# ShannonAI/GNN-LM

Hardware: AMD Instinct MI355X
Metric: eval tokens/sec on WikiText-103 (k=1024, GNN+KNN); test ppl match (higher is better)
Workload: dtype f32

## Files before the change

### gnn-lm_amd/csrc/ivfpq_mfma.hip

```cpp
#include "kernels.h"

namespace gnnlm {
namespace {

typedef int v4i __attribute__((ext_vector_type(4)));
typedef int v8i __attribute__((ext_vector_type(8)));
typedef unsigned u32x2 __attribute__((ext_vector_type(2)));
typedef unsigned v4u __attribute__((ext_vector_type(4)));
constexpr int QG = 8;
constexpr int TAB_BYTES = 2 * 256 * 32 * QG;
#ifndef GNNLM_IVF8_WAVE_CAP
#define GNNLM_IVF8_WAVE_CAP 240
#endif
constexpr int WAVE_CAP = GNNLM_IVF8_WAVE_CAP;
constexpr int SCAN_CTL = 768;
constexpr int SCAN_LDS = TAB_BYTES + SCAN_CTL + 16 * WAVE_CAP * 8;
static_assert(SCAN_LDS <= 160 * 1024, "the filter's tables + staging regions exceed a CU's LDS");
constexpr int HIST_BINS = 1024, HIST_SHIFT = 4;
constexpr int SUMS_LDS = TAB_BYTES + QG * HIST_BINS * 4;
constexpr int SURV_CNT_STRIDE = 16;
constexpr int QLUT_BYTES = 64 * 256;
constexpr int SURV_ROW_BITS = 19, SURV_LIST_BITS = 18, SURV_EXCESS_MAX = 254, SURV_SUM_BIG = 16383;

__global__ __launch_bounds__(256) void pack_tiles_kernel(const uint8_t* __restrict__ codes, int64_t N, uint8_t* __restrict__ out) {
// ... 381 lines not shown
                    const uint32_t t0 = GNNLM_PERM(b, a, 0x05010400u), t1 = GNNLM_PERM(b, a, 0x07030602u);
                    const uint32_t t2 = GNNLM_PERM(d, c, 0x05010400u), t3 = GNNLM_PERM(d, c, 0x07030602u);
                    o[0 + hq] = GNNLM_PERM(t2, t0, 0x05040100u);
                    o[2 + hq] = GNNLM_PERM(t2, t0, 0x07060302u);
                    o[4 + hq] = GNNLM_PERM(t3, t1, 0x05040100u);
                    o[6 + hq] = GNNLM_PERM(t3, t1, 0x07060302u);
                }
                uint4* dst = reinterpret_cast<uint4*>(smem) + 2 * (tid + (i0 + it) * NTH);
                dst[0] = uint4{o[0], o[1], o[2], o[3]};
                dst[1] = uint4{o[4], o[5], o[6], o[7]};
            }
        }
    }
#endif
    const int j = lane & 15, g = lane >> 4;
    const int qs_lane = lane < QG ? gq[lane] : -1;
    uint32_t* hist = reinterpret_cast<uint32_t*>(smem + TAB_BYTES);
    if (SUMS) for (int e = tid; e < QG * HIST_BINS; e += NTH) hist[e] = 0u;
    constexpr int T_NEVER = 16384;
    int T4[4] = {T_NEVER, T_NEVER, T_NEVER, T_NEVER};
    uint32_t *hist_a = nullptr, *hist_b = nullptr;
    if (SUMS) {
        const int q0 = 4 * (g & 1) + (g >= 2 ? 2 : 0) + (j & 1), q1 = q0 ^ 1;
        if (gq[q0] >= 0 && p.grp_out[(int64_t)grp * QG + q0] >= 0) hist_a = hist + q0 * HIST_BINS;
        if (gq[q1] >= 0 && p.grp_out[(int64_t)grp * QG + q1] >= 0) hist_b = hist + q1 * HIST_BINS;
    } else if (g < 2) {
#pragma unroll
        for (int r = 0; r < 4; ++r) {
            const int qr = gq[4 * g + r];
            if (qr >= 0) T4[r] = max(-T_NEVER, min(T_NEVER, filter_threshold(p.qmeta, qr, p.coarse[(int64_t)qr * p.ld_coarse + list], p.tau[qr])));
        }
    }
#if GNNLM_IVF8_EXP & 32
    if (p.cap > 0) T4[0] = T4[1] = T4[2] = T4[3] = T_NEVER;
#elif GNNLM_IVF8_EXP & 255
    T4[0] = T4[1] = T4[2] = T4[3] = T_NEVER;
#endif
    if (!SUMS && wave == 0) {
        int Tl = 0;
#pragma unroll
        for (int sl = 0; sl < QG; ++sl) {
            const int t = __builtin_amdgcn_readlane(T4[sl & 3], 16 * (sl >> 2));
            if (lane == sl) Tl = t;
        }
        if (lane < QG) { wgc[lane] = 0; wgc[8 + lane] = Tl; wgc[16 + lane] = qs_lane; }
    }
    const v4i negT = SUMS ? v4i{0, 0, 0, 0} : v4i{1 - T4[0], 1 - T4[1], 1 - T4[2], 1 - T4[3]};
    __syncthreads();
    phase(0);
#if GNNLM_IVF8_EXP & 1024
    const long long g0 = clock64();
#endif

    uint32_t tc[8];
#pragma unroll
    for (int s = 0; s < 8; ++s) {
        const uint32_t s0 = (uint32_t)(16 * (g & 1) + ((j + 2 * s) & 15)) << 3, s1 = (uint32_t)(16 * (g & 1) + ((j + 2 * s + 1) & 15)) << 3;
        tc[s] = s0 | s1 << 8 | (uint32_t)(g >> 1) << 16;
    }
    uint32_t sel[4] = {0u, 0u, 0u, 0u}, sidx = 0xccccccccu;
    if (j < QG) {
        const int pos = j & 3;
#pragma unroll
        for (int h = 0; h < 2; ++h)
#pragma unroll
            for (int lk = 0; lk < 2; ++lk) {
                const int s0 = 8 * h + 2 * (2 * lk + (j >> 2));
                const int sb = pos < 3 ? s0 : s0 + 1;
                sel[sb >> 2] |= 1u << (8 * (sb & 3));
                if (pos < 3) sidx = (sidx & ~(3u << (2 * s0))) | (uint32_t)pos << (2 * s0);
            }
    }
    const v4i Asel = {(int)sel[0], (int)sel[1], (int)sel[2], (int)sel[3]};

    const int64_t t_lo = lo >> 4;
    const int nt = (int)(((hi - 1) >> 4) - t_lo) + 1;
    const int len = (int)(hi - lo), row_shift = (int)(lo & 15);
    const __amdgpu_buffer_rsrc_t rs = __builtin_amdgcn_make_buffer_rsrc(const_cast<uint8_t*>(p.tiles) + t_lo * 1024, 0, nt * 1024, 0x00020000);
    const int wv = __builtin_amdgcn_readfirstlane(wave);
    const int voff = lane * 16;
    const uint32_t rs_lane = (uint32_t)((j - row_shift) * 8) + (uint32_t)(4 * (g & 1));
    auto load_tile = [&](int u) -> v4u {
#if GNNLM_IVF8_EXP & 1
        return v4u{(uint32_t)u * 2654435761u + lane, (uint32_t)u * 40503u ^ lane, (uint32_t)u + 77u * lane, (uint32_t)u * 3u + lane};
#elif GNNLM_IVF8_EXP & 256
        return __builtin_amdgcn_raw_buffer_load_b128(rs, voff, __builtin_amdgcn_readfirstlane((u & 3) * 1024), 0);
#else
        return __builtin_amdgcn_raw_buffer_load_b128(rs, voff, __builtin_amdgcn_readfirstlane(u * 1024), 0);
#endif
    };
    auto lookups4 = [&](const v4u& cw, int q, v8i& X) __attribute__((always_inline)) {
        const uint32_t w[4] = {cw.x, cw.y, cw.z, cw.w};
#pragma unroll
        for (int e = 0; e < 4; ++e) {
            const int pp = 4 * q + e;
            const uint32_t ad = GNNLM_PERM(w[pp >> 2], tc[pp >> 1], 0x0c020000u | (uint32_t)(4 + (pp & 3)) << 8 | (uint32_t)(pp & 1));
#if GNNLM_IVF8_EXP & 4
            const u32x2 x = u32x2{ad, ad ^ 0x55u};
#else
            const u32x2 x = *reinterpret_cast<const __attribute__((address_space(3))) u32x2*>(ad);
#endif
            X[2 * e] = (int)x.x;
            X[2 * e + 1] = (int)x.y;
        }
    };
    int wcnt = 0;
    auto count_entries = [&](int* ctr) __attribute__((always_inline)) {
        for (int c = lane; c < wcnt; c += 64) {
            const uint2 e = wbuf[c];
#pragma unroll
            for (int r = 0; r < 4; ++r)
                if (e.y >> (8 * r) & 255u) atomicAdd(&ctr[(e.x & 4u) + r], 1);
        }
    };
    auto write_entries = [&](int* pos) __attribute__((always_inline)) {
        for (int c = lane; c < wcnt; c += 64) {
            const uint2 e = wbuf[c];
            const uint32_t row = (uint32_t)(lo + ((e.x >> 3) & ((1u << SURV_ROW_BITS) - 1u)));
#pragma unroll
            for (int r = 0; r < 4; ++r) {
                const int b8 = (int)(e.y >> (8 * r) & 255u);
                if (b8 == 0) continue;
                const int sl = (int)(e.x & 4u) + r;
                const int64_t at = atomicAdd(&pos[sl], 1);
                const int Tsl = wgc[8 + sl], qsl = wgc[16 + sl];
                if (at < p.cap && qsl >= 0) {
                    const int ex = b8 - 1;
                    const int su = ex >= SURV_EXCESS_MAX ? SURV_SUM_BIG : min(SURV_SUM_BIG - 1, max(0, ex + Tsl + 128 * 64));
                    surv[(int64_t)qsl * p.cap + at] = uint2{row, (uint32_t)list | (uint32_t)su << SURV_LIST_BITS};
                }
            }
        }
        wcnt = 0;
    };
    auto flush_wave = [&]() __attribute__((always_inline)) {
        if (wcnt == 0) return;
        if (lane < QG) wc[lane] = 0;
        count_entries(wc);
        if (lane < QG) {
            const int tot = wc[lane];
            wc[lane] = (tot > 0 && qs_lane >= 0) ? atomicAdd(&p.surv_cnt[(int64_t)qs_lane * SURV_CNT_STRIDE], tot) : 0;
        }
        write_entries(wc);
    };
    constexpr int PF = SUMS ? GNNLM_IVF8_PF_SUMS : GNNLM_IVF8_PF;
    v8i X[4];
    const int TS = SUMS ? max(1, p.sums_stride) : 1;
    auto step = [&](const v4u& cn, v4u& cl, int u) __attribute__((always_inline)) {
        tick(-1);
        cl = load_tile(u + PF * NW * TS);
        v4i acc = negT;
#pragma unroll
        for (int q = 0; q < 4; ++q) {
#if GNNLM_IVF8_EXP & 8
            acc += v4i{X[q][0], X[q][1], X[q][2], X[q][3]} + v4i{X[q][4], X[q][5], X[q][6], X[q][7]};
#else
            acc = __builtin_amdgcn_smfmac_i32_16x16x128_i8(Asel, X[q], acc, (int)sidx, 0, 0);
#endif
            lookups4(cn, q, X[q]);
            __builtin_amdgcn_sched_barrier(0);
        }
        tick(0);
        const int row = 16 * u + j - row_shift;
        const bool edge = u == 0 || u >= nt - 1;
        if (SUMS) {
            const gnnlm_u32x2 w2 = __builtin_amdgcn_permlane32_swap((uint32_t)acc[2], (uint32_t)acc[2], false, false);
            const gnnlm_u32x2 w3 = __builtin_amdgcn_permlane32_swap((uint32_t)acc[3], (uint32_t)acc[3], false, false);
            const int e0 = g >= 2 ? (int)w2.x : acc[0], e1 = g >= 2 ? (int)w3.x : acc[1];
            const int s0 = (j & 1) ? e1 : e0, s1 = (j & 1) ? e0 : e1;
            if (!edge || (unsigned)row < (unsigned)len) {
                if (hist_a) atomicAdd(&hist_a[(s0 + 128 * 64) >> HIST_SHIFT], 1u);
                if (hist_b) atomicAdd(&hist_b[(s1 + 128 * 64) >> HIST_SHIFT], 1u);
            }
        } else {
            if (wcnt + 32 > WAVE_CAP) flush_wave();
            tick(1);
            uint32_t lo8, hi8;
            const uint32_t p01 = GNNLM_PERM((uint32_t)acc[1], (uint32_t)acc[0], 0x05040100u), p23 = GNNLM_PERM((uint32_t)acc[3], (uint32_t)acc[2], 0x05040100u);
            asm("v_sat_pk_u8_i16 %0, %1" : "=v"(lo8) : "v"(p01));
            asm("v_sat_pk_u8_i16 %0, %1" : "=v"(hi8) : "v"(p23));
            const uint32_t ex4 = GNNLM_PERM(hi8, lo8, 0x05040100u);
            const uint32_t rowslot = ((uint32_t)(16 * u) << 3) + rs_lane;
            const uint32_t lim = edge ? (uint32_t)len << 3 : 0xffffffffu;
            uint32_t ex4r = rowslot < lim ? ex4 : 0u;
            asm("" : "+v"(ex4r));
            const bool keep = ex4r != 0u;
            const uint64_t m = __builtin_amdgcn_ballot_w64(keep);
            const int rank = __builtin_amdgcn_mbcnt_hi((uint32_t)(m >> 32), __builtin_amdgcn_mbcnt_lo((uint32_t)m, 0u));
            if (keep) wbuf[wcnt + rank] = uint2{rowslot, ex4r};
            wcnt = __builtin_amdgcn_readfirstlane(wcnt + __builtin_popcountll(m));
            tick(2);
        }
    };
    {
        int u = SUMS ? wv * TS + list % TS : wv;
        v4u C[PF];
#pragma unroll
        for (int i = 0; i < PF; ++i) C[i] = load_tile(u + i * NW * TS);
#pragma unroll
        for (int q = 0; q < 4; ++q) lookups4(C[0], q, X[q]);
#define GNNLM_IVF8_STEP(t) if constexpr (PF > (t)) { step(C[((t) + 1) % PF], C[(t)], u); u += NW * TS; }
        while (u < nt) {
            GNNLM_IVF8_STEP(0) GNNLM_IVF8_STEP(1) GNNLM_IVF8_STEP(2) GNNLM_IVF8_STEP(3)
            GNNLM_IVF8_STEP(4) GNNLM_IVF8_STEP(5) GNNLM_IVF8_STEP(6) GNNLM_IVF8_STEP(7)
        }
#undef GNNLM_IVF8_STEP
        static_assert(PF >= 3 && PF <= 8, "GNNLM_IVF8_PF");
        phase(1);
#if GNNLM_IVF8_EXP & 512
        if (tid == 512 && p.work_ctr) for (int i = 0; i < 3; ++i) { atomicAdd(&p.work_ctr[(blockIdx.x & 7) * 16 + 8 + i], acc_t[i]); acc_t[i] = 0; }
        if (tid == 512 && p.work_ctr) atomicAdd(&p.work_ctr[(blockIdx.x & 7) * 16 + 11], (nt - wv + NW - 1) / NW);
#endif
#if GNNLM_IVF8_EXP & 1024
        if (lane == 0 && p.work_ctr) atomicAdd(&p.work_ctr[(blockIdx.x & 7) * 16 + (wave ? wave : 15)], (int)((clock64() - g0) >> 4));
#endif
    }
    if (SUMS) {
        __syncthreads();
#pragma unroll
        for (int u = 0; u < QG; ++u) {
            const int64_t ob = p.grp_out[(int64_t)grp * QG + u];
            if (qs[u] < 0 || ob < 0) continue;
            for (int e = tid; e < HIST_BINS; e += NTH) p.out_hist[ob + e] = hist[u * HIST_BINS + e];
        }
        advance_slow();
        continue;
    }
    count_entries(wgc);
    if (tid == 0) *next_s = next_index();
    phase(3);
    __syncthreads();
    phase(4);
    if (tid < QG) {
        const int tot = wgc[tid];
        wgc[tid] = (tot > 0 && qs_lane >= 0) ? atomicAdd(&p.surv_cnt[(int64_t)qs_lane * SURV_CNT_STRIDE], tot) : 0;
    }
    __syncthreads();
    gi_next = *next_s;
    phase(5);
    write_entries(wgc);
    }
#if GNNLM_IVF8_EXP & 512
    if (tid == 0 && p.work_ctr) {
        atomicAdd(&p.work_ctr[(blockIdx.x & 7) * 16 + 12], (int)((clock64() - k0) >> 4));
        atomicAdd(&p.work_ctr[(blockIdx.x & 7) * 16 + 13], (int)(wall_clock64() - w0));
    }
#endif
}

__global__ __launch_bounds__(1024) void ivfpq_tau_kernel(gnnlm_ivfpq_tau_t p) {
    constexpr int CB = 2 * HIST_BINS;
    __shared__ int comb[CB];
    __shared__ int part[1024];
    __shared__ int bstar_s;
    const int tid = threadIdx.x;
    const int64_t q = blockIdx.x;
    const float delta = p.qmeta[q * 4], sum_lo = p.qmeta[q * 4 + 1], amax = p.qmeta[q * 4 + 2];
    float bmin = INFINITY, bmax = -INFINITY;
    for (int d = 0; d < p.D; ++d) {
        if (p.probe_list[q * p.ld_probe + d] < 0) continue;
        const float b = p.probe_bias[q * p.ld_probe + d];
        bmin = fminf(bmin, b);
        bmax = fmaxf(bmax, b);
    }
    int c0 = 0, c1 = 0;
    for (int d = 0; d < p.D; ++d) {
        if (p.probe_list[q * p.ld_probe + d] < 0) continue;
        const float offf = (p.probe_bias[q * p.ld_probe + d] - bmin) / delta * 0.9999f - 1.f;
        const int sh = (int)fminf(fmaxf(offf, 0.f), (float)(HIST_BINS << HIST_SHIFT)) >> HIST_SHIFT;
        const uint32_t* h = p.hist + (q * p.D + d) * HIST_BINS;
        const int b0 = tid - sh, b1 = tid + 1024 - sh;
        if (b0 >= 0 && b0 < HIST_BINS) c0 += (int)h[b0];
        if (b1 >= 0 && b1 < HIST_BINS) c1 += (int)h[b1];
    }
    comb[tid] = c0;
    comb[tid + 1024] = c1;
    if (tid == 0) bstar_s = -1;
    __syncthreads();
    const int h0 = comb[2 * tid], h1 = comb[2 * tid + 1], mine = h0 + h1;
    part[tid] = mine;
    __syncthreads();
    int suf = mine;
    for (int step = 1; step < 1024; step <<= 1) {
        const int other = tid + step < 1024 ? part[tid + step] : 0;
        __syncthreads();
        suf += other;
        part[tid] = suf;
        __syncthreads();
    }
    if (suf >= p.k && suf - mine < p.k) bstar_s = (suf - mine + h1 >= p.k) ? 2 * tid + 1 : 2 * tid;
    __syncthreads();
    if (tid == 0) {
        float tau = -INFINITY;
        if (bstar_s >= 0) {
            const float eps = 66.f * 2.3841858e-7f * (64.f * amax + fmaxf(fabsf(bmin), fabsf(bmax)));
            tau = (bmin + sum_lo) + (float)(bstar_s << HIST_SHIFT) * delta * (1.f - 6.1035156e-5f) - eps;
            tau -= fabsf(tau) * 2.3841858e-7f + 1e-30f;
        }
        p.tau[q] = tau;
    }
}

#ifndef GNNLM_REFINE_NT
#define GNNLM_REFINE_NT 1024
#endif
struct RefineParams {
    uint32_t* surv;  const int32_t* surv_cnt;  int32_t* out_cnt;  int32_t cap;
    float* tau;  const float* qmeta;
    const float* coarse;  int64_t ld_coarse;
    int64_t n;  int32_t k;
};
template <int EPT>
__device__ __forceinline__ void refine_wg(const RefineParams& p, const int64_t q, int* hist, int& n_left, float& tau_left) {
    constexpr int NT = GNNLM_REFINE_NT, NB = 2048, NWV = NT / 64;
    __shared__ int wtot[NWV];
    __shared__ int dig_s, base_s;
    const int tid = threadIdx.x, lane = tid & 63, wave = tid >> 6;
    const int n = min(p.surv_cnt[q * SURV_CNT_STRIDE], p.cap);
    uint2* surv = reinterpret_cast<uint2*>(p.surv) + q * p.cap;
    const float tau0 = p.tau[q];
    n_left = n;
    tau_left = tau0;
    if (n < p.k || !(tau0 > -INFINITY)) {
        if (tid == 0 && p.out_cnt) p.out_cnt[q * SURV_CNT_STRIDE] = n;
        return;
    }
    const float delta = p.qmeta[q * 4], sum_lo = p.qmeta[q * 4 + 1], amax = p.qmeta[q * 4 + 2];
    const float dlo = delta * (1.f - 6.1035156e-5f);
    const float* coarse = p.coarse + q * p.ld_coarse;
    auto lower_bound = [&](const uint2& rec) -> float {
        const int list = (int)(rec.y & ((1u << SURV_LIST_BITS) - 1u));
        int su = (int)(rec.y >> SURV_LIST_BITS);
        const float bias = coarse[list];
        if (su >= SURV_SUM_BIG) su = min(16320, max(0, filter_threshold(p.qmeta, q, bias, tau0) + SURV_EXCESS_MAX + 128 * 64));
        const float eps = 66.f * 2.3841858e-7f * (64.f * amax + fabsf(bias));
        const float lb = (bias + sum_lo) + (float)su * dlo - eps;
        return lb - (fabsf(lb) * 2.3841858e-7f + 1e-30f);
    };
    constexpr int C0 = EPT * NT;
    uint2 rrec[EPT];
    float rlb[EPT];
#pragma unroll
    for (int e = 0; e < EPT; ++e) rrec[e] = surv[min(tid + e * NT, n - 1)];
    float mx = -INFINITY;
#pragma unroll
    for (int e = 0; e < EPT; ++e) {
        rlb[e] = tid + e * NT < n ? lower_bound(rrec[e]) : -INFINITY;
        mx = fmaxf(mx, rlb[e]);
    }
    for (int c = C0 + tid; c < n; c += NT) mx = fmaxf(mx, lower_bound(surv[c]));
    __shared__ float wmax[NWV];
    mx = wave_max(mx);
    if (lane == 0) wmax[wave] = mx;
    __syncthreads();
    mx = wmax[0];
    for (int w = 1; w < NWV; ++w) mx = fmaxf(mx, wmax[w]);
    const float span = mx - tau0;
    float tau1 = tau0;
    if (span > 0.f) {
        const float inv_w = (float)NB / span * (1.f - 1e-6f);
        for (int e = tid; e < NB; e += NT) hist[e] = 0;
        __syncthreads();
        auto bin_of = [&](float lb) -> int { return lb >= tau0 ? min(NB - 1, (int)((lb - tau0) * inv_w)) : -1; };
#pragma unroll
        for (int e = 0; e < EPT; ++e) {
            const int bn = bin_of(rlb[e]);
            if (bn >= 0) atomicAdd(&hist[bn], 1);
        }
        for (int c = C0 + tid; c < n; c += NT) {
            const int bn = bin_of(lower_bound(surv[c]));
            if (bn >= 0) atomicAdd(&hist[bn], 1);
        }
        __syncthreads();
        constexpr int BPT = NB / NT;
        int own[BPT], mine = 0;
#pragma unroll
        for (int bb = 0; bb < BPT; ++bb) { own[bb] = hist[BPT * tid + bb]; mine += own[bb]; }
        int suf = mine;
#pragma unroll
        for (int d = 1; d < 64; d <<= 1) {
            const int o = __shfl_down(suf, d, 64);
            if (lane + d < 64) suf += o;
        }
        if (lane == 0) wtot[wave] = suf;
        if (tid == 0) dig_s = -1;
        __syncthreads();
        for (int w = wave + 1; w < NWV; ++w) suf += wtot[w];
        if (suf >= p.k && suf - mine < p.k) {
            int acc_ = suf - mine;
#pragma unroll
            for (int bb = BPT - 1; bb >= 0; --bb) {
                if (acc_ + own[bb] >= p.k) { dig_s = BPT * tid + bb; break; }
                acc_ += own[bb];
            }
        }
        __syncthreads();
        if (dig_s > 0) {
            const float t = tau0 + (float)dig_s / inv_w * (1.f - 2e-6f);
            tau1 = fmaxf(tau0, t - fabsf(t) * 4.7683716e-7f);
        }
    }
    auto keep_rec = [&](const uint2& rec) -> bool {
        const int list = (int)(rec.y & ((1u << SURV_LIST_BITS) - 1u)), su = (int)(rec.y >> SURV_LIST_BITS);
        if (su >= SURV_SUM_BIG) return true;
        const float bias = coarse[list];
        const float eps = 66.f * 2.3841858e-7f * (64.f * amax + fabsf(bias) + fabsf(tau1));
        const float ub = (bias + sum_lo) + (float)(su + 66) * delta * 1.001f + eps;
        return !(ub < tau1);
    };
    int kept = 0;
    uint32_t kmask = 0u;
#pragma unroll
    for (int e = 0; e < EPT; ++e)
        if (tid + e * NT < n && keep_rec(rrec[e])) { kmask |= 1u << e; ++kept; }
    int incl = kept;
#pragma unroll
    for (int d = 1; d < 64; d <<= 1) {
        const int o = __shfl_up(incl, d, 64);
        if (lane >= d) incl += o;
    }
    __syncthreads();
    if (lane == 63) wtot[wave] = incl;
    __syncthreads();
    int at = incl - kept;
    for (int w = 0; w < wave; ++w) at += wtot[w];
    int total = 0;
    for (int w = 0; w < NWV; ++w) total += wtot[w];
#pragma unroll
    for (int e = 0; e < EPT; ++e)
        if (kmask >> e & 1u) surv[at++] = rrec[e];
    if (n > C0) {
        if (tid == 0) base_s = total;
        __syncthreads();
        for (int c0 = C0; c0 < n; c0 += NT) {
            const int c = c0 + tid;
            uint2 rec = uint2{0u, 0u};
            bool keep = false;
            if (c < n) { rec = surv[c]; keep = keep_rec(rec); }
            const uint64_t m = __builtin_amdgcn_ballot_w64(keep);
            const int rank = __builtin_amdgcn_mbcnt_hi((uint32_t)(m >> 32), __builtin_amdgcn_mbcnt_lo((uint32_t)m, 0u));
            __syncthreads();
            if (lane == 0) wtot[wave] = __builtin_popcountll(m);
            __syncthreads();
            int before = base_s;
            for (int w = 0; w < wave; ++w) before += wtot[w];
            if (keep) surv[before + rank] = rec;
            __syncthreads();
            if (tid == 0) { int tot = 0; for (int w = 0; w < NWV; ++w) tot += wtot[w]; base_s += tot; }
            __syncthreads();
        }
        total = base_s;
    }
    if (tid == 0) {
        if (p.out_cnt) p.out_cnt[q * SURV_CNT_STRIDE] = total;
        p.tau[q] = tau1;
    }
    n_left = total;
    tau_left = tau1;
}

#ifndef GNNLM_RESCORE_NT
#define GNNLM_RESCORE_NT 1024
#endif
template <int M, bool TAB_READY>
__device__ __forceinline__ void rescore_wg(const gnnlm_ivfpq_rescore_t& p, const int64_t q, const int n, const float tau, float* rtab) {
    __shared__ int ccnt;
    constexpr int NT = GNNLM_RESCORE_NT;
    uint32_t* cdw = reinterpret_cast<uint32_t*>(rtab + M * 256);
    const int tid = threadIdx.x;
#ifdef GNNLM_RESCORE_DBG
    long long dbg_t = clock64(); int dbg_i = 0;
    auto dbg = [&]() { const long long t = clock64(); if (tid == 0) reinterpret_cast<int*>(p.cand_val + (q + 1) * p.cand_cap - 8)[dbg_i] = (int)(t - dbg_t); ++dbg_i; dbg_t = t; };
#else
    auto dbg = [&]() {};
#endif
    if (tid == 0) ccnt = 0;
    const uint2* surv = reinterpret_cast<const uint2*>(p.surv) + q * p.cap;
    const int last = max(n - 1, 0);
    auto record = [&](int e, uint2& rec) __attribute__((always_inline)) { rec = surv[min(e, last)]; };
    auto rowload = [&](const uint2& rec, v4u (&cr)[M / 16], float& bias) __attribute__((always_inline)) {
        bias = p.coarse[q * p.ld_coarse + (rec.y & ((1u << SURV_LIST_BITS) - 1u))];
        const v4u* crow = reinterpret_cast<const v4u*>(p.codes + (int64_t)rec.x * M);
#pragma unroll
        for (int c16 = 0; c16 < M / 16; ++c16) cr[c16] = crow[c16];
    };
    uint2 recC = uint2{0u, 0u}, recD = recC;
    v4u cr0[M / 16], cr1[M / 16];
    float bias0 = 0.f, bias1 = 0.f;
    uint32_t rid0 = 0u, rid1 = 0u;
    if (n > 0) {
        if (!TAB_READY) {
            const float4* src = reinterpret_cast<const float4*>(p.lut + q * p.ld_lut);
            float4* dst = reinterpret_cast<float4*>(rtab);
            for (int e = tid; e < M * 64; e += NT) dst[e] = src[e];
        }
        uint2 r0, r1;
        record(tid, r0);
        record(tid + NT, r1);
        record(tid + 2 * NT, recC);
        rowload(r0, cr0, bias0);
        rid0 = r0.x;
        rowload(r1, cr1, bias1);
        rid1 = r1.x;
    }
    dbg();
    __syncthreads();
    dbg();
    const uint8_t* cb = reinterpret_cast<const uint8_t*>(cdw + tid);
    auto one = [&](int e, v4u (&cr)[M / 16], float& bset, uint32_t& rset, const uint2& rec_old, uint2& rec_new) __attribute__((always_inline)) {
        const int64_t row = rset;
        const float bias = bset;
#pragma unroll
        for (int c16 = 0; c16 < M / 16; ++c16) {
            cdw[(4 * c16 + 0) * NT + tid] = cr[c16].x;
            cdw[(4 * c16 + 1) * NT + tid] = cr[c16].y;
            cdw[(4 * c16 + 2) * NT + tid] = cr[c16].z;
            cdw[(4 * c16 + 3) * NT + tid] = cr[c16].w;
        }
        record(e + 3 * NT, rec_new);
        rowload(rec_old, cr, bset);
        rset = rec_old.x;
        const int rot = (int)(row & 31);
        float a0 = 0.f, a1 = 0.f;
#pragma unroll
        for (int h = 0; h < M / 32; ++h) {
#pragma unroll 8
            for (int s = 0; s < 32; s += 2) {
                const int m0 = 32 * h + ((rot + s) & 31), m1 = 32 * h + ((rot + s + 1) & 31);
                a0 = a0 + rtab[m0 * 256 + cb[(m0 >> 2) * (4 * NT) + (m0 & 3)]];
                a1 = a1 + rtab[m1 * 256 + cb[(m1 >> 2) * (4 * NT) + (m1 & 3)]];
            }
        }
        const float score = bias + (a0 + a1);
        if (score > tau) {
            const int pos = atomicAdd(&ccnt, 1);
            if (pos < p.cand_cap) {
                p.cand_val[q * p.cand_cap + pos] = score;
                p.cand_id[q * p.cand_cap + pos] = row;
            }
        }
    };
    int e = tid;
#pragma unroll
    for (int it = 0; it < 8; ++it) {
        if (e >= n) break;
        one(e, cr0, bias0, rid0, recC, recD);
        e += NT;
        if (e >= n) break;
        one(e, cr1, bias1, rid1, recD, recC);
        e += NT;
    }
    for (; e < n; e += 2 * NT) {
        one(e, cr0, bias0, rid0, recC, recD);
        if (e + NT >= n) break;
        one(e + NT, cr1, bias1, rid1, recD, recC);
    }
    dbg();
    __syncthreads();
    dbg();
    if (tid == 0) p.cand_cnt[q] = ccnt;
    const int nc = min(ccnt, p.cand_cap);
    for (int e = tid; e < nc; e += NT) p.cand_id[q * p.cand_cap + e] = p.payload[p.cand_id[q * p.cand_cap + e]];
    dbg();
}

template <int M>
__global__ __launch_bounds__(GNNLM_RESCORE_NT) void ivfpq_rescore_kernel(gnnlm_ivfpq_rescore_t p) {
    extern __shared__ __attribute__((aligned(16))) float rtab[];
    const int64_t q = blockIdx.x;
    rescore_wg<M, false>(p, q, min(p.surv_cnt[q * SURV_CNT_STRIDE], p.cap), p.tau[q], rtab);
}

static_assert(GNNLM_REFINE_NT == GNNLM_RESCORE_NT, "the fused refine + re-score launch runs both on one workgroup shape");
template <int EPT>
__global__ __launch_bounds__(GNNLM_RESCORE_NT) void ivfpq_refine_rescore_kernel(gnnlm_ivfpq_rescore_t p) {
    constexpr int M = 64;
    extern __shared__ __attribute__((aligned(16))) float rtab[];
    const int tid = threadIdx.x, lane = tid & 63, wave = tid >> 6;
    const int64_t q = blockIdx.x;
    const int n0 = min(p.surv_cnt[q * SURV_CNT_STRIDE], p.cap);
    if (n0 > 0) {
        const float* src = p.lut + q * p.ld_lut + (4 * wave) * 256 + 4 * lane;
        const unsigned dst = (unsigned)(uintptr_t)(__attribute__((address_space(3))) void*)rtab + (unsigned)(4 * __builtin_amdgcn_readfirstlane(wave)) * 1024u;
        unsigned keep_;
        asm volatile("s_mov_b32 %0, m0\n\ts_mov_b32 m0, %2\n\ts_nop 0\n\t"
                     "global_load_lds_dwordx4 %1, off\n\tglobal_load_lds_dwordx4 %1, off offset:1024\n\t"
                     "global_load_lds_dwordx4 %1, off offset:2048\n\tglobal_load_lds_dwordx4 %1, off offset:3072\n\t"
                     "s_mov_b32 m0, %0"
                     : "=&s"(keep_) : "v"(src), "s"(dst) : "memory");
    }
    RefineParams r;
    r.surv = const_cast<uint32_t*>(p.surv);  r.surv_cnt = p.surv_cnt;  r.out_cnt = p.out_cnt;  r.cap = p.cap;
    r.tau = const_cast<float*>(p.tau);  r.qmeta = p.qmeta;  r.coarse = p.coarse;  r.ld_coarse = p.ld_coarse;  r.n = p.n;  r.k = p.k;
    int n_left;
    float tau_left;
    refine_wg<EPT>(r, q, reinterpret_cast<int*>(rtab + M * 256), n_left, tau_left);
    asm volatile("s_waitcnt vmcnt(0)" ::: "memory");
    __syncthreads();
    rescore_wg<M, true>(p, q, n_left, tau_left, rtab);
}

}

int ivfpq_pack_tiles(const uint8_t* codes, int64_t N, int M, uint8_t* out, hipStream_t stream) {
    GNNLM_REQUIRE(codes && out && N >= 0 && M == 64, "ivfpq_pack_tiles: need M = 64");
    GNNLM_REQUIRE((uintptr_t)out % 16 == 0, "ivfpq_pack_tiles: 16-byte aligned output");
    const int64_t threads = ((N + 15) >> 4 << 4) * 4;
    if (threads == 0) return OK;
    GNNLM_REQUIRE(cdiv(threads, (int64_t)256) < (1ll << 31), "ivfpq_pack_tiles: too many rows for one launch");
    hipLaunchKernelGGL(pack_tiles_kernel, dim3((unsigned)cdiv(threads, (int64_t)256)), dim3(256), 0, stream, codes, N, out);
    GNNLM_LAUNCH_CHECK();
    return OK;
}

int ivfpq_build_groups(const int64_t* pl, int64_t ld, int64_t n, int P, int nlist, int64_t seg, int32_t* grp_list, int32_t* grp_q,
                       int64_t* grp_out, int32_t* n_groups, int32_t* scratch, hipStream_t stream) {
    GNNLM_REQUIRE(n >= 0 && P > 0 && nlist > 0 && n * P < (1ll << 31) && ld >= P, "ivfpq_build_groups: bad shape");
    GNNLM_REQUIRE(pl && grp_list && grp_q && n_groups && scratch, "ivfpq_build_groups: null operand");
    const int64_t G = n * P / QG + nlist + 1, pairs = n * P;
    const int64_t fill = std::max<int64_t>(G * QG, 2 * (int64_t)(nlist + 1));
    hipLaunchKernelGGL(groups_fill_kernel, dim3((unsigned)cdiv(fill, (int64_t)256)), dim3(256), 0, stream, grp_list, grp_q, grp_out, G, scratch, nlist);
    if (pairs > 0)
        hipLaunchKernelGGL(groups_count_kernel, dim3((unsigned)cdiv(pairs, (int64_t)256)), dim3(256), 0, stream, pl, ld, n, P, nlist, scratch);
    hipLaunchKernelGGL(groups_scan_kernel, dim3(1), dim3(1024), 0, stream, scratch, nlist, n_groups);
    if (pairs > 0)
        hipLaunchKernelGGL(groups_scatter_kernel, dim3((unsigned)cdiv(pairs, (int64_t)256)), dim3(256), 0, stream, pl, ld, n, P, nlist, seg, scratch,
                           scratch + nlist + 1, grp_list, grp_q, grp_out);
    GNNLM_LAUNCH_CHECK();
    return OK;
}

int ivfpq_quantize_lut(const float* lut, int64_t ld_lut, int64_t n, int M, uint8_t* qlut, float* qmeta, hipStream_t stream) {
    GNNLM_REQUIRE(lut && qlut && qmeta && n >= 0 && n < (1ll << 31) && M == 64 && ld_lut >= 64 * 256 && ld_lut % 4 == 0 &&
                      (uintptr_t)lut % 16 == 0 && (uintptr_t)qlut % 16 == 0,
                  "ivfpq_quantize_lut: need M = 64 and 16-byte aligned tables");
    if (n == 0) return OK;
    hipLaunchKernelGGL(quantize_lut_kernel, dim3((unsigned)n), dim3(256), 0, stream, lut, ld_lut, qlut, qmeta);
    GNNLM_LAUNCH_CHECK();
    return OK;
}

int ivfpq_tables(const gnnlm_ivfpq_tables_t& d, hipStream_t stream) {
    GNNLM_REQUIRE(d.qr && d.pq && d.lut && d.qlut && d.qmeta && d.n >= 0 && d.n < (1ll << 31), "ivfpq_tables: null operand or bad n");
    GNNLM_REQUIRE(d.M == 64 && (d.dsub == 4 || d.dsub == 8 || d.dsub == 16 || d.dsub == 32),
                  "ivfpq_tables: need M = 64 and dsub in {4, 8, 16, 32} (other shapes: gnnlm_gemm_nt + gnnlm_ivfpq_quantize_lut)");
    GNNLM_REQUIRE(d.ld_qr >= 64 * d.dsub && d.ld_qr % 4 == 0 && d.ld_lut >= 64 * 256 && d.ld_lut % 4 == 0 &&
                      (uintptr_t)d.qr % 16 == 0 && (uintptr_t)d.pq % 16 == 0 && (uintptr_t)d.lut % 16 == 0 &&
                      (uintptr_t)d.qlut % 16 == 0 && (uintptr_t)d.qmeta % 16 == 0,
                  "ivfpq_tables: rows of qr / lut must be 16-byte aligned and hold 64 * dsub / 64 * 256 floats");
    if (d.n == 0) return OK;
    const dim3 grid((unsigned)cdiv(d.n, (int64_t)TQ));
#define GNNLM_TABLES_LAUNCH(DS)                                                                                 \
    GNNLM_LDS_OPT_IN(&ivfpq_tables_kernel<DS>, TABLES_LDS);                                                     \
    hipLaunchKernelGGL(ivfpq_tables_kernel<DS>, grid, dim3(256), TABLES_LDS, stream, d);
    if (d.dsub == 4) { GNNLM_TABLES_LAUNCH(4) }
    else if (d.dsub == 8) { GNNLM_TABLES_LAUNCH(8) }
    else if (d.dsub == 16) { GNNLM_TABLES_LAUNCH(16) }
    else { GNNLM_TABLES_LAUNCH(32) }
#undef GNNLM_TABLES_LAUNCH
    GNNLM_LAUNCH_CHECK();
    return OK;
}

int ivfpq_scan8(const gnnlm_ivfpq_scan8_t& d, hipStream_t stream) {
    GNNLM_REQUIRE(d.max_groups >= 0, "ivfpq_scan8: bad group count");
    if (d.max_groups == 0) return OK;
    GNNLM_REQUIRE(d.tiles && d.list_off && d.qlut && d.qmeta && d.coarse && d.grp_list && d.grp_q && d.n_groups &&
                      (d.out_hist || (d.tau && d.surv && d.surv_cnt && d.cap > 0)),
                  "ivfpq_scan8: null operand");
    GNNLM_REQUIRE(d.M == 64 && (uintptr_t)d.tiles % 16 == 0 && (uintptr_t)d.qlut % 4 == 0, "ivfpq_scan8: need M = 64, aligned images");
    GNNLM_REQUIRE(!d.out_hist || d.grp_out, "ivfpq_scan8: out_hist needs grp_out");
    GNNLM_REQUIRE(d.nlist > 0 && d.nlist <= (1 << SURV_LIST_BITS) && d.max_list >= 0 && d.max_list < (1ll << SURV_ROW_BITS),
                  "ivfpq_scan8: the survivor records hold 18 bits of list and 19 bits of row: need 0 < nlist <= 2^18 and max_list < 2^19");
    GNNLM_LDS_OPT_IN(&ivfpq_scan8_kernel<false>, SCAN_LDS);
    GNNLM_LDS_OPT_IN(&ivfpq_scan8_kernel<true>, SUMS_LDS);
    ProfScope prof(d.out_hist ? K_IVF8S : K_IVF8, stream, 0.0, 0.0);
    int dev = 0, cus = 0;
    GNNLM_HIP(hipGetDevice(&dev));
    GNNLM_HIP(hipDeviceGetAttribute(&cus, hipDeviceAttributeMultiprocessorCount, dev));
    const int64_t grid = std::min<int64_t>(8 * cdiv((int64_t)d.max_groups, (int64_t)8), 8 * cdiv((int64_t)std::max(cus, 8), (int64_t)8));
    if (d.out_hist) hipLaunchKernelGGL(ivfpq_scan8_kernel<true>, dim3((unsigned)grid), dim3(NTH), SUMS_LDS, stream, d);
    else hipLaunchKernelGGL(ivfpq_scan8_kernel<false>, dim3((unsigned)grid), dim3(NTH), SCAN_LDS, stream, d);
    GNNLM_LAUNCH_CHECK();
    return OK;
}

int ivfpq_tau(const gnnlm_ivfpq_tau_t& d, hipStream_t stream) {
    GNNLM_REQUIRE(d.n >= 0 && d.n < (1ll << 31) && d.D >= 1 && d.k > 0, "ivfpq_tau: bad shape");
    if (d.n == 0) return OK;
    GNNLM_REQUIRE(d.hist && d.probe_list && d.probe_bias && d.qmeta && d.tau && d.ld_probe >= d.D, "ivfpq_tau: null operand");
    ProfScope prof(K_TAU, stream, 0.0, 4.0 * (double)d.n * d.D * HIST_BINS);
    hipLaunchKernelGGL(ivfpq_tau_kernel, dim3((unsigned)d.n), dim3(1024), 0, stream, d);
    GNNLM_LAUNCH_CHECK();
    return OK;
}

__global__ __launch_bounds__(256) void split_payload_kernel(int64_t* __restrict__ idx, int64_t n, int label_bits, int32_t val_last, int32_t* __restrict__ out_vals) {
    const int64_t e = (int64_t)blockIdx.x * 256 + threadIdx.x;
    if (e >= n) return;
    const int64_t v = idx[e];
    idx[e] = v < 0 ? v : v >> label_bits;
    if (out_vals) out_vals[e] = v < 0 ? val_last : (int32_t)(v & ((1ll << label_bits) - 1));
}
int ivfpq_split_payload(int64_t* idx, int64_t n, int label_bits, int32_t val_last, int32_t* out_vals, hipStream_t stream) {
    GNNLM_REQUIRE(idx && n >= 0 && label_bits > 0 && label_bits < 32, "ivfpq_split_payload: bad arguments");
    if (n == 0) return OK;
    hipLaunchKernelGGL(split_payload_kernel, dim3((unsigned)cdiv(n, (int64_t)256)), dim3(256), 0, stream, idx, n, label_bits, val_last, out_vals);
    GNNLM_LAUNCH_CHECK();
    return OK;
}

int ivfpq_rescore(const gnnlm_ivfpq_rescore_t& d, hipStream_t stream) {
    GNNLM_REQUIRE(d.n >= 0 && d.n < (1ll << 31), "ivfpq_rescore: bad query count");
    if (d.n == 0) return OK;
    GNNLM_REQUIRE(d.codes && d.payload && d.lut && d.coarse && d.tau && d.surv && d.surv_cnt && d.cand_val && d.cand_id && d.cand_cnt &&
                      d.cap > 0 && d.cand_cap > 0,
                  "ivfpq_rescore: null operand");
    GNNLM_REQUIRE(d.M == 64 && d.ld_lut >= (int64_t)d.M * 256 && d.ld_lut % 4 == 0 && (uintptr_t)d.lut % 16 == 0 &&
                      (uintptr_t)d.codes % 16 == 0,
                  "ivfpq_rescore: need M = 64, 16-byte aligned tables");
    ProfScope prof(K_RESCORE, stream, 0.0, 0.0);
    const size_t lds = (size_t)d.M * 256 * 4 + GNNLM_RESCORE_NT * (size_t)d.M;
    if (d.qmeta) {
        GNNLM_REQUIRE(d.k > 0, "ivfpq_rescore: the refinement needs k > 0");
        GNNLM_LDS_OPT_IN(&ivfpq_refine_rescore_kernel<8>, lds);
        hipLaunchKernelGGL(ivfpq_refine_rescore_kernel<8>, dim3((unsigned)d.n), dim3(GNNLM_RESCORE_NT), lds, stream, d);
        GNNLM_LAUNCH_CHECK();
        return OK;
    }
    GNNLM_LDS_OPT_IN(&ivfpq_rescore_kernel<64>, lds);
    hipLaunchKernelGGL(ivfpq_rescore_kernel<64>, dim3((unsigned)d.n), dim3(GNNLM_RESCORE_NT), lds, stream, d);
    GNNLM_LAUNCH_CHECK();
    return OK;
}

}
```

Measured before the change: 560,600.

## Keep PQ codes in registers and halve rescore workgroup for two blocks per CU

Rescore used to stage each candidate's 64 code bytes through an LDS transpose buffer. Now it rotates them in registers with select/alignbyte and builds table offsets with byte perms, which drops the staging LDS. With that LDS gone and workgroups cut from 1024 to 512 threads, two workgroups fit per CU; the refine EPT and the LUT preload are rescaled to match. Scheduling barriers and a straight-line unrolled loop are added, at the cost of more VALU work per lookup and higher register pressure.

```diff
diff --git a/gnn-lm_amd/csrc/ivfpq_mfma.hip b/gnn-lm_amd/csrc/ivfpq_mfma.hip
--- a/gnn-lm_amd/csrc/ivfpq_mfma.hip
+++ b/gnn-lm_amd/csrc/ivfpq_mfma.hip
@@ -707,7 +707,7 @@
 }
 
 #ifndef GNNLM_REFINE_NT
-#define GNNLM_REFINE_NT 1024
+#define GNNLM_REFINE_NT 512
 #endif
 struct RefineParams {
     uint32_t* surv;  const int32_t* surv_cnt;  int32_t* out_cnt;  int32_t cap;
@@ -752,6 +752,7 @@
     for (int e = 0; e < EPT; ++e) {
         rlb[e] = tid + e * NT < n ? lower_bound(rrec[e]) : -INFINITY;
         mx = fmaxf(mx, rlb[e]);
+        if (e % 4 == 3) __builtin_amdgcn_sched_barrier(0);
     }
     for (int c = C0 + tid; c < n; c += NT) mx = fmaxf(mx, lower_bound(surv[c]));
     __shared__ float wmax[NWV];
@@ -816,8 +817,10 @@
     int kept = 0;
     uint32_t kmask = 0u;
 #pragma unroll
-    for (int e = 0; e < EPT; ++e)
+    for (int e = 0; e < EPT; ++e) {
         if (tid + e * NT < n && keep_rec(rrec[e])) { kmask |= 1u << e; ++kept; }
+        if (e % 4 == 3) __builtin_amdgcn_sched_barrier(0);
+    }
     int incl = kept;
 #pragma unroll
     for (int d = 1; d < 64; d <<= 1) {
@@ -865,13 +868,25 @@
 }
 
 #ifndef GNNLM_RESCORE_NT
-#define GNNLM_RESCORE_NT 1024
-#endif
+#define GNNLM_RESCORE_NT 512
+#endif
+static_assert(GNNLM_RESCORE_NT == 512 || GNNLM_RESCORE_NT == 1024, "the re-score's workgroup: 8 or 16 waves");
+constexpr int RESCORE_TAB_LDS = 64 * 256 * 4;
+constexpr int REFINE_HIST_LDS = 2048 * 4;
+constexpr int RESCORE_STATIC_LDS = 256;
+static_assert(2 * (RESCORE_TAB_LDS + REFINE_HIST_LDS + RESCORE_STATIC_LDS) <= 160 * 1024 && RESCORE_TAB_LDS + REFINE_HIST_LDS + RESCORE_STATIC_LDS <= 80 * 1024,
+              "two workgroups of the re-score per CU");
+template <int K, class F>
+__device__ __forceinline__ void straight_line(F& f) {
+    if constexpr (K > 0) {
+        if (f()) straight_line<K - 1>(f);
+    }
+}
 template <int M, bool TAB_READY>
 __device__ __forceinline__ void rescore_wg(const gnnlm_ivfpq_rescore_t& p, const int64_t q, const int n, const float tau, float* rtab) {
+    static_assert(M == 64, "two halves of 32 sub-quantizers");
     __shared__ int ccnt;
     constexpr int NT = GNNLM_RESCORE_NT;
-    uint32_t* cdw = reinterpret_cast<uint32_t*>(rtab + M * 256);
     const int tid = threadIdx.x;
 #ifdef GNNLM_RESCORE_DBG
     long long dbg_t = clock64(); int dbg_i = 0;
@@ -911,29 +926,45 @@
     dbg();
     __syncthreads();
     dbg();
-    const uint8_t* cb = reinterpret_cast<const uint8_t*>(cdw + tid);
+    const char* tabb = reinterpret_cast<const char*>(rtab);
     auto one = [&](int e, v4u (&cr)[M / 16], float& bset, uint32_t& rset, const uint2& rec_old, uint2& rec_new) __attribute__((always_inline)) {
         const int64_t row = rset;
         const float bias = bset;
-#pragma unroll
-        for (int c16 = 0; c16 < M / 16; ++c16) {
-            cdw[(4 * c16 + 0) * NT + tid] = cr[c16].x;
-            cdw[(4 * c16 + 1) * NT + tid] = cr[c16].y;
-            cdw[(4 * c16 + 2) * NT + tid] = cr[c16].z;
-            cdw[(4 * c16 + 3) * NT + tid] = cr[c16].w;
+        const uint32_t rot = (uint32_t)row & 31u, rb = rot & 3u;
+        const bool r4 = rot & 16u, r2 = rot & 8u, r1 = rot & 4u;
+        uint32_t f[2][8];
+#pragma unroll
+        for (int h = 0; h < 2; ++h) {
+            const uint32_t d[8] = {cr[2 * h].x, cr[2 * h].y, cr[2 * h].z, cr[2 * h].w, cr[2 * h + 1].x, cr[2 * h + 1].y, cr[2 * h + 1].z, cr[2 * h + 1].w};
+            uint32_t t4[8], t2[8], t1[8];
+            auto sel = [](bool c, uint32_t a, uint32_t b) __attribute__((always_inline)) -> uint32_t { return c ? a : b; };
+#pragma unroll
+            for (int i = 0; i < 8; ++i) t4[i] = sel(r4, d[(i + 4) & 7], d[i]);
+#pragma unroll
+            for (int i = 0; i < 8; ++i) t2[i] = sel(r2, t4[(i + 2) & 7], t4[i]);
+#pragma unroll
+            for (int i = 0; i < 8; ++i) t1[i] = sel(r1, t2[(i + 1) & 7], t2[i]);
+#pragma unroll
+            for (int i = 0; i < 8; ++i) f[h][i] = __builtin_amdgcn_alignbyte(t1[(i + 1) & 7], t1[i], rb);
         }
         record(e + 3 * NT, rec_new);
         rowload(rec_old, cr, bset);
         rset = rec_old.x;
-        const int rot = (int)(row & 31);
+        uint32_t J[8];
+#pragma unroll
+        for (int i = 0; i < 8; ++i) J[i] = (rot * 0x01010101u + (0x03020100u + 0x04040404u * (uint32_t)i)) & 0x1f1f1f1fu;
+        auto lookup = [&](int h, int s) __attribute__((always_inline)) -> float {
+            const uint32_t sel = 0x0c0c0000u | (uint32_t)(4 + (s & 3)) << 8 | (uint32_t)(s & 3);
+            const uint32_t at = __builtin_amdgcn_perm(J[s >> 2], f[h][s >> 2], sel) << 2;
+            return *reinterpret_cast<const float*>(tabb + (h << 15) + at);
+        };
         float a0 = 0.f, a1 = 0.f;
 #pragma unroll
-        for (int h = 0; h < M / 32; ++h) {
-#pragma unroll 8
+        for (int h = 0; h < 2; ++h) {
+#pragma unroll
             for (int s = 0; s < 32; s += 2) {
-                const int m0 = 32 * h + ((rot + s) & 31), m1 = 32 * h + ((rot + s + 1) & 31);
-                a0 = a0 + rtab[m0 * 256 + cb[(m0 >> 2) * (4 * NT) + (m0 & 3)]];
-                a1 = a1 + rtab[m1 * 256 + cb[(m1 >> 2) * (4 * NT) + (m1 & 3)]];
+                a0 = a0 + lookup(h, s);
+                a1 = a1 + lookup(h, s + 1);
             }
         }
         const float score = bias + (a0 + a1);
@@ -946,15 +977,16 @@
         }
     };
     int e = tid;
-#pragma unroll
-    for (int it = 0; it < 8; ++it) {
-        if (e >= n) break;
+    auto two = [&]() __attribute__((always_inline)) -> bool {
+        if (e >= n) return false;
         one(e, cr0, bias0, rid0, recC, recD);
         e += NT;
-        if (e >= n) break;
+        if (e >= n) return false;
         one(e, cr1, bias1, rid1, recD, recC);
         e += NT;
-    }
+        return true;
+    };
+    straight_line<16384 / (2 * NT)>(two);
     for (; e < n; e += 2 * NT) {
         one(e, cr0, bias0, rid0, recC, recD);
         if (e + NT >= n) break;
@@ -969,30 +1001,36 @@
     dbg();
 }
 
+constexpr int RESCORE_WAVES_PER_SIMD = 4;
 template <int M>
-__global__ __launch_bounds__(GNNLM_RESCORE_NT) void ivfpq_rescore_kernel(gnnlm_ivfpq_rescore_t p) {
+__global__ __launch_bounds__(GNNLM_RESCORE_NT, RESCORE_WAVES_PER_SIMD) void ivfpq_rescore_kernel(gnnlm_ivfpq_rescore_t p) {
     extern __shared__ __attribute__((aligned(16))) float rtab[];
     const int64_t q = blockIdx.x;
     rescore_wg<M, false>(p, q, min(p.surv_cnt[q * SURV_CNT_STRIDE], p.cap), p.tau[q], rtab);
 }
 
 static_assert(GNNLM_REFINE_NT == GNNLM_RESCORE_NT, "the fused refine + re-score launch runs both on one workgroup shape");
+constexpr int REFINE_EPT = 8192 / GNNLM_REFINE_NT;
 template <int EPT>
-__global__ __launch_bounds__(GNNLM_RESCORE_NT) void ivfpq_refine_rescore_kernel(gnnlm_ivfpq_rescore_t p) {
-    constexpr int M = 64;
+__global__ __launch_bounds__(GNNLM_RESCORE_NT, RESCORE_WAVES_PER_SIMD) void ivfpq_refine_rescore_kernel(gnnlm_ivfpq_rescore_t p) {
+    constexpr int M = 64, PIECES = 64 / (GNNLM_RESCORE_NT / 64);
     extern __shared__ __attribute__((aligned(16))) float rtab[];
     const int tid = threadIdx.x, lane = tid & 63, wave = tid >> 6;
     const int64_t q = blockIdx.x;
     const int n0 = min(p.surv_cnt[q * SURV_CNT_STRIDE], p.cap);
     if (n0 > 0) {
-        const float* src = p.lut + q * p.ld_lut + (4 * wave) * 256 + 4 * lane;
-        const unsigned dst = (unsigned)(uintptr_t)(__attribute__((address_space(3))) void*)rtab + (unsigned)(4 * __builtin_amdgcn_readfirstlane(wave)) * 1024u;
-        unsigned keep_;
-        asm volatile("s_mov_b32 %0, m0\n\ts_mov_b32 m0, %2\n\ts_nop 0\n\t"
-                     "global_load_lds_dwordx4 %1, off\n\tglobal_load_lds_dwordx4 %1, off offset:1024\n\t"
-                     "global_load_lds_dwordx4 %1, off offset:2048\n\tglobal_load_lds_dwordx4 %1, off offset:3072\n\t"
-                     "s_mov_b32 m0, %0"
-                     : "=&s"(keep_) : "v"(src), "s"(dst) : "memory");
+#pragma unroll
+        for (int g = 0; g < PIECES / 4; ++g) {
+            const float* src = p.lut + q * p.ld_lut + (PIECES * wave + 4 * g) * 256 + 4 * lane;
+            const unsigned dst = (unsigned)(uintptr_t)(__attribute__((address_space(3))) void*)rtab +
+                                 (unsigned)(PIECES * __builtin_amdgcn_readfirstlane(wave) + 4 * g) * 1024u;
+            unsigned keep_;
+            asm volatile("s_mov_b32 %0, m0\n\ts_mov_b32 m0, %2\n\ts_nop 0\n\t"
+                         "global_load_lds_dwordx4 %1, off\n\tglobal_load_lds_dwordx4 %1, off offset:1024\n\t"
+                         "global_load_lds_dwordx4 %1, off offset:2048\n\tglobal_load_lds_dwordx4 %1, off offset:3072\n\t"
+                         "s_mov_b32 m0, %0"
+                         : "=&s"(keep_) : "v"(src), "s"(dst) : "memory");
+        }
     }
     RefineParams r;
     r.surv = const_cast<uint32_t*>(p.surv);  r.surv_cnt = p.surv_cnt;  r.out_cnt = p.out_cnt;  r.cap = p.cap;
@@ -1125,16 +1163,15 @@
                       (uintptr_t)d.codes % 16 == 0,
                   "ivfpq_rescore: need M = 64, 16-byte aligned tables");
     ProfScope prof(K_RESCORE, stream, 0.0, 0.0);
-    const size_t lds = (size_t)d.M * 256 * 4 + GNNLM_RESCORE_NT * (size_t)d.M;
     if (d.qmeta) {
         GNNLM_REQUIRE(d.k > 0, "ivfpq_rescore: the refinement needs k > 0");
-        GNNLM_LDS_OPT_IN(&ivfpq_refine_rescore_kernel<8>, lds);
-        hipLaunchKernelGGL(ivfpq_refine_rescore_kernel<8>, dim3((unsigned)d.n), dim3(GNNLM_RESCORE_NT), lds, stream, d);
+        GNNLM_LDS_OPT_IN(&ivfpq_refine_rescore_kernel<REFINE_EPT>, RESCORE_TAB_LDS + REFINE_HIST_LDS);
+        hipLaunchKernelGGL(ivfpq_refine_rescore_kernel<REFINE_EPT>, dim3((unsigned)d.n), dim3(GNNLM_RESCORE_NT), RESCORE_TAB_LDS + REFINE_HIST_LDS, stream, d);
         GNNLM_LAUNCH_CHECK();
         return OK;
     }
-    GNNLM_LDS_OPT_IN(&ivfpq_rescore_kernel<64>, lds);
-    hipLaunchKernelGGL(ivfpq_rescore_kernel<64>, dim3((unsigned)d.n), dim3(GNNLM_RESCORE_NT), lds, stream, d);
+    GNNLM_LDS_OPT_IN(&ivfpq_rescore_kernel<64>, RESCORE_TAB_LDS);
+    hipLaunchKernelGGL(ivfpq_rescore_kernel<64>, dim3((unsigned)d.n), dim3(GNNLM_RESCORE_NT), RESCORE_TAB_LDS, stream, d);
     GNNLM_LAUNCH_CHECK();
     return OK;
 }
```

Result: no change. 565,900, median of 6 (+0.9%).
